# gau-nernst/llama-x

Hardware: AMD Instinct MI355X
Metric: train tokens/sec Llama-3.1-8B seq4096 at 1/2/4/8 MI355X; p50 step ms (higher is better)
Workload: dtype bf16; 1 GPU; Llama-3.1-8B text-only LoRA r=16 bf16, seq=4096, 1 sequence per GPU, causal mask, base+LM head frozen (BASELINE.json configs[1]); random-init weights at 8B dimensions; seq_len=4096, parallelism=dp1, launch=hipGraph replay (fwd+bwd+AdamW), lm_head_rows=labelled only

## Files before the change

llama-x_amd/csrc/attn.h:

```cpp
#pragma once
#include "common.h"
#include <type_traits>

#define BQ 128
#define BKV 64
#define TILE_BYTES (64 * HD * 2)

typedef __attribute__((address_space(3))) void lds_void;
typedef const __attribute__((address_space(1))) void gbl_void;
typedef __attribute__((address_space(3))) s16x4_t lds_s16x4;

static inline int attn_check_shape(const char* fn, int64_t B, int64_t S, int64_t H, int64_t KVH, int64_t head_dim) {
  LLX_REQUIRE(head_dim == HD, "%s: head_dim=%lld unsupported (only 128)", fn, (long long)head_dim);
  LLX_REQUIRE(B > 0 && S > 0 && H > 0 && KVH > 0 && H % KVH == 0, "%s: bad B/S/H/KVH", fn);
  return LLX_OK;
}
int attn_dropout_check(const char* fn, int64_t threshold, const void* rng, int64_t stream_id, int64_t B, int64_t H);
template <typename... K>
static inline hipError_t attn_lds_limit(int bytes, K... kernels) {
  hipError_t e = hipSuccess;
  for (const void* f : {(const void*)kernels...}) if (e == hipSuccess) e = hipFuncSetAttribute(f, hipFuncAttributeMaxDynamicSharedMemorySize, bytes);
  return e;
}
```

llama-x_amd/csrc/attn_bwd.hip:

```cpp
#include "attn.h"
#include "attn_dropout.h"

typedef __attribute__((ext_vector_type(8))) short s16x8_t;

__device__ __forceinline__ int dual_swz(int row) { return ((row & 3) << 2) | ((row >> 2) & 3); }
__device__ __forceinline__ uint32_t dual_swz(uint32_t row) { return ((row & 3) << 2) | ((row >> 2) & 3); }

__device__ __forceinline__ bf16x8_t tr_frag(const char* img, int row0, int db, int lane) {
  const int hh = lane >> 5, tq = (lane & 15) >> 2, tp = lane & 3, tsub = (lane >> 4) & 1;
  const int chunk = 4 * db + 2 * tsub + (tp >> 1);
  const int rlo = row0 + 4 * hh + tq, rhi = rlo + 8;
  s16x4_t lo = __builtin_amdgcn_ds_read_tr16_b64_v4i16((lds_s16x4*)(img + rlo * 256 + ((chunk ^ dual_swz(rlo)) << 4) + ((tp & 1) << 3)));
  s16x4_t hi = __builtin_amdgcn_ds_read_tr16_b64_v4i16((lds_s16x4*)(img + rhi * 256 + ((chunk ^ dual_swz(rhi)) << 4) + ((tp & 1) << 3)));
  s16x8_t v = {lo[0], lo[1], lo[2], lo[3], hi[0], hi[1], hi[2], hi[3]};
  return __builtin_bit_cast(bf16x8_t, v);
}

__device__ __forceinline__ bf16x8_t row_frag(const char* img, int row, int ks, int hh) {
  return *reinterpret_cast<const bf16x8_t*>(img + row * 256 + (((2 * ks + hh) ^ dual_swz(row)) << 4));
}

template <int N>
__device__ __forceinline__ void lds_tr_wait(s16x4_t& a, s16x4_t& b, s16x4_t (&c)[4], s16x4_t (&d)[4]) {
  asm volatile("s_waitcnt lgkmcnt(%10)"
               : "+v"(a), "+v"(b), "+v"(c[0]), "+v"(c[1]), "+v"(c[2]), "+v"(c[3]), "+v"(d[0]), "+v"(d[1]), "+v"(d[2]), "+v"(d[3])
               : "n"(N));
  __builtin_amdgcn_sched_barrier(0);
}
__device__ __forceinline__ uint32_t xor_imm(uint32_t a, int c) {
  if (c == 0) return a;
  uint32_t r;
  asm volatile("v_xor_b32 %0, %1, %2" : "=v"(r) : "n"(c), "v"(a));
  return r;
}

struct AttnBwdArgs {
  const bf16_t* q; const bf16_t* k; const bf16_t* v; const bf16_t* o; const bf16_t* d_o;
  const float* lse; float* delta; float* nlse;
  const float* rope;
  unsigned long long* stamps;
  bf16_t* dq; bf16_t* dk; bf16_t* dv;
  bf16_t* ds; int Sp;
  int64_t q_sb, q_ss, k_sb, k_ss, v_sb, v_ss, o_sb, o_ss, do_sb, do_ss;
  int64_t dq_sb, dq_ss, dk_sb, dk_ss, dv_sb, dv_ss;
  const int* doc_ids; const int* prefix_len; const uint8_t* flags;
  int B, S, H, KVH;
  float scale, scale_log2;
  const uint8_t* mask; int64_t m_sb, m_sq;
  const int64_t* rng; uint32_t drop_thr; float drop_c; int stream_id;
};

enum { BWD_CAUSAL = 0, BWD_RULE = 1, BWD_MASK = 2 };

__device__ __forceinline__ uint32_t mask_nibble(uint32_t w) {
  const uint32_t nz = (((w & 0x7f7f7f7fu) + 0x7f7f7f7fu) | w) & 0x80808080u;
  return ((nz >> 7) * 0x01020408u) >> 24;
}

#define DQ_STAGE_BYTES (2 * TILE_BYTES)
#define DQ_LDS_BYTES (2 * DQ_STAGE_BYTES)

template <int MODE, bool DROPOUT = false>
__global__ __launch_bounds__(256, 2) void attn_bwd_dq_kernel(const AttnBwdArgs a) {
  static_assert(!(DROPOUT && MODE == BWD_MASK), "dropout exists in the causal and the rule mode");
  constexpr bool GENERAL = MODE == BWD_RULE;
  constexpr bool FLAGS = MODE != BWD_CAUSAL;
  constexpr bool MASK = MODE == BWD_MASK;
  extern __shared__ __attribute__((aligned(256))) char smem[];
  const int tid = threadIdx.x, lane = tid & 63;
  const int wave = __builtin_amdgcn_readfirstlane(tid >> 6);
  const int nqb = (a.S + BQ - 1) / BQ, nkt = (a.S + BKV - 1) / BKV;
  const int qb = nqb - 1 - blockIdx.y;
  const int h = blockIdx.x, b = blockIdx.z;
  const int kvh = h / (a.H / a.KVH);
  const int r = lane & 31, hh = lane >> 5;
  const int qi = qb * BQ + wave * 32 + r;
  const int qrow = min(qi, a.S - 1);

  const uint8_t* fl = FLAGS ? a.flags + ((int64_t)b * nqb + qb) * nkt : nullptr;
  const int kt_end = FLAGS ? nkt : min(nkt, (qb * BQ + BQ + BKV - 1) / BKV);
  uint32_t fpack = 0;
  int fchunk = -1;
  auto tile_class = [&](int t) -> int {
    if constexpr (FLAGS) {
      if ((t >> 6) != fchunk) {
        fchunk = t >> 6;
        fpack = fl[min(fchunk * 64 + lane, nkt - 1)];
      }
      return __builtin_amdgcn_readlane((int)fpack, t & 63);
    } else {
      return (t * BKV + BKV - 1 <= qb * BQ) ? 2 : 1;
    }
  };
  auto next_tile = [&](int t) {
    while (t < kt_end && tile_class(t) == 0) ++t;
    return t;
  };

  const int srow_in = lane >> 4, sslot = lane & 15;
  const bf16_t* kbase = a.k + (int64_t)b * a.k_sb + kvh * HD;
  const bf16_t* vbase = a.v + (int64_t)b * a.v_sb + kvh * HD;
  uint32_t koff[4], voff[4];
#pragma unroll
  for (int i = 0; i < 4; ++i) {
    const int row = i * 16 + wave * 4 + srow_in;
    koff[i] = (uint32_t)(((int64_t)row * a.k_ss + (sslot ^ dual_swz(row)) * 8) * 2);
    voff[i] = (uint32_t)(((int64_t)row * a.v_ss + (sslot ^ (row & 15)) * 8) * 2);
  }
  auto stage = [&](int buf, int t) {
    char* sK = smem + buf * DQ_STAGE_BYTES;
    char* sV = sK + TILE_BYTES;
    if (t * BKV + BKV <= a.S) {
      const char* kt = (const char*)(kbase + (int64_t)t * BKV * a.k_ss);
      const char* vt = (const char*)(vbase + (int64_t)t * BKV * a.v_ss);
      if constexpr (DROPOUT) {
        uint32_t l0;
        asm volatile("v_mbcnt_lo_u32_b32 %0, -1, 0\n\tv_mbcnt_hi_u32_b32 %0, -1, %0" : "=v"(l0));
        const int slot = (int)(l0 & 15);
#pragma unroll
        for (int i = 0; i < 4; ++i) {
          const int row = i * 16 + wave * 4 + (int)(l0 >> 4);
          const uint32_t ko = (uint32_t)(((int64_t)row * a.k_ss + (slot ^ dual_swz(row)) * 8) * 2);
          const uint32_t vo = (uint32_t)(((int64_t)row * a.v_ss + (slot ^ (row & 15)) * 8) * 2);
          __builtin_amdgcn_global_load_lds((gbl_void*)(kt + ko), (lds_void*)(sK + (i * 16 + wave * 4) * 256), 16, 0, 0);
          __builtin_amdgcn_global_load_lds((gbl_void*)(vt + vo), (lds_void*)(sV + (i * 16 + wave * 4) * 256), 16, 0, 0);
        }
      } else {
#pragma unroll
      for (int i = 0; i < 4; ++i) {
        __builtin_amdgcn_global_load_lds((gbl_void*)(kt + koff[i]), (lds_void*)(sK + (i * 16 + wave * 4) * 256), 16, 0, 0);
        __builtin_amdgcn_global_load_lds((gbl_void*)(vt + voff[i]), (lds_void*)(sV + (i * 16 + wave * 4) * 256), 16, 0, 0);
      }
      }
    } else {
#pragma unroll
      for (int i = 0; i < 4; ++i) {
        const int row = i * 16 + wave * 4 + srow_in;
        const int key = min(t * BKV + row, a.S - 1);
        const int kc = sslot ^ dual_swz(row);
        const int vc = sslot ^ (row & 15);
        __builtin_amdgcn_global_load_lds((gbl_void*)(kbase + (int64_t)key * a.k_ss + kc * 8), (lds_void*)(sK + (i * 16 + wave * 4) * 256), 16, 0, 0);
        __builtin_amdgcn_global_load_lds((gbl_void*)(vbase + (int64_t)key * a.v_ss + vc * 8), (lds_void*)(sV + (i * 16 + wave * 4) * 256), 16, 0, 0);
      }
    }
  };

  const uint32_t sbase = (uint32_t)(uintptr_t)(__attribute__((address_space(3))) char*)smem;
  uint32_t aK0;
  {
    const int tq2 = (lane & 15) >> 2, tp = lane & 3, tsub = (lane >> 4) & 1;
    const int rlo = 4 * hh + tq2;
    aK0 = (uint32_t)(rlo * 256 + (((2 * tsub + (tp >> 1)) ^ dual_swz(rlo)) << 4) + ((tp & 1) << 3));
  }
  f32x16_t dq[4];
#pragma unroll
  for (int i = 0; i < 4; ++i)
#pragma unroll
    for (int e = 0; e < 16; ++e) dq[i][e] = 0.f;
  const int* docrow = (GENERAL && a.doc_ids) ? a.doc_ids + (int64_t)b * a.S : nullptr;
  const int my_doc = docrow ? docrow[qrow] : 0;
  const int my_prefix = (GENERAL && a.prefix_len) ? a.prefix_len[b] : 0;
  uint32_t mwn[MASK ? 8 : 1];
  auto mask_request = [&](int t_) {
    if constexpr (MASK) {
      uint32_t l0;
      asm volatile("v_mbcnt_lo_u32_b32 %0, -1, 0\n\tv_mbcnt_hi_u32_b32 %0, -1, %0" : "=v"(l0));
      const int hh = (int)(l0 >> 5);
      const uint8_t* mrow = a.mask + (int64_t)b * a.m_sb + (int64_t)min(qb * BQ + wave * 32 + (int)(l0 & 31), a.S - 1) * a.m_sq;
      if (t_ * BKV + BKV <= a.S) {
        const uint8_t* p = mrow + t_ * BKV + 4 * hh;
#pragma unroll
        for (int g = 0; g < 8; ++g) __builtin_memcpy(&mwn[g], p + (g >> 2) * 32 + 8 * (g & 3), 4);
      } else {
#pragma unroll
        for (int g = 0; g < 8; ++g) {
          const int g0 = t_ * BKV + (g >> 2) * 32 + 8 * (g & 3) + 4 * hh;
          __builtin_memcpy(&mwn[g], mrow + min(g0, a.S - 4), 4);
        }
      }
    }
  };
  auto mask_bits = [&](int t_) -> uint32_t {
    uint32_t bits = 0;
    if constexpr (MASK) {
      const bool ragged = t_ * BKV + BKV > a.S;
#pragma unroll
      for (int g = 0; g < 8; ++g) {
        uint32_t w = mwn[g];
        if (ragged) {
          const int g0 = t_ * BKV + (g >> 2) * 32 + 8 * (g & 3) + 4 * hh;
          const int sh = g0 - min(g0, a.S - 4);
          w = sh >= 4 ? 0u : w >> (8 * sh);
        }
        bits |= mask_nibble(w) << (4 * g);
      }
    }
    return bits;
  };

  int t = next_tile(0);
  if constexpr (MASK) {
#pragma unroll
    for (int g = 0; g < 8; ++g) mwn[g] = 0;
    if (t < kt_end && tile_class(t) == 1) mask_request(t);
  }
  if (t < kt_end) stage(0, t);
  bf16x8_t qf[8], dof[8], ovf[8];
  const float my_lse = a.lse[((int64_t)b * a.H + h) * a.S + qrow];
  {
    const bf16_t* qp = a.q + (int64_t)b * a.q_sb + (int64_t)qrow * a.q_ss + h * HD + 8 * hh;
    const bf16_t* dp = a.d_o + (int64_t)b * a.do_sb + (int64_t)qrow * a.do_ss + h * HD + 8 * hh;
    const bf16_t* op = a.o + (int64_t)b * a.o_sb + (int64_t)qrow * a.o_ss + h * HD + 8 * hh;
#pragma unroll
    for (int ks = 0; ks < 8; ++ks) {
      ovf[ks] = *reinterpret_cast<const bf16x8_t*>(op + 16 * ks);
      dof[ks] = *reinterpret_cast<const bf16x8_t*>(dp + 16 * ks);
      qf[ks] = *reinterpret_cast<const bf16x8_t*>(qp + 16 * ks);
    }
    __builtin_amdgcn_sched_barrier(0);
  }
  const float lse_safe = (my_lse == -INFINITY) ? 0.f : my_lse;
// ... 752 lines not shown
  return (2 * B * H * S + (H / KVH) * 2 * B * S * KVH * HD) * 4;
}

extern "C" int64_t llx_attn_bwd_ds_bytes(int64_t B, int64_t S, int64_t H) {
  const int64_t Sp = cdiv64(S, 256) * 256;
  return B * H * Sp * Sp * 2;
}

static int attn_bwd_set_attrs() {
  static const hipError_t e0 = attn_lds_limit(DQ_LDS_BYTES, attn_bwd_dq_kernel<BWD_CAUSAL>, attn_bwd_dq_kernel<BWD_RULE>, attn_bwd_dq_kernel<BWD_MASK>,
                                              attn_bwd_dq_kernel<BWD_CAUSAL, true>, attn_bwd_dq_kernel<BWD_RULE, true>);
  static const hipError_t e1 = attn_lds_limit(DQ2_LDS_BYTES, attn_bwd_dq2_kernel<false>, attn_bwd_dq2_kernel<true>);
  static const hipError_t e2 = attn_lds_limit(DKV3_LDS_BYTES, attn_bwd_dkv3_kernel<BWD_CAUSAL, false, false>, attn_bwd_dkv3_kernel<BWD_RULE, false, false>,
                                              attn_bwd_dkv3_kernel<BWD_MASK, false, false>, attn_bwd_dkv3_kernel<BWD_CAUSAL, true, false>,
                                              attn_bwd_dkv3_kernel<BWD_CAUSAL, false, true>, attn_bwd_dkv3_kernel<BWD_RULE, false, true>,
                                              attn_bwd_dkv3_kernel<BWD_CAUSAL, false, false, true>, attn_bwd_dkv3_kernel<BWD_RULE, false, false, true>);
  return e0 == hipSuccess && e1 == hipSuccess && e2 == hipSuccess ? LLX_OK : LLX_ERR_LAUNCH;
}

static int attn_bwd_args(const char* fn, AttnBwdArgs& a, const void* q, int64_t q_sb, int64_t q_ss, const void* k, int64_t k_sb, int64_t k_ss,
                         const void* v, int64_t v_sb, int64_t v_ss, const void* o, int64_t o_sb, int64_t o_ss, const void* d_o, int64_t do_sb,
                         int64_t do_ss, const float* lse, float* delta, void* dq, int64_t dq_sb, int64_t dq_ss, void* dk, int64_t dk_sb,
                         int64_t dk_ss, void* dv, int64_t dv_sb, int64_t dv_ss, const float* rope, int64_t B, int64_t S, int64_t H, int64_t KVH,
                         int64_t head_dim, float scale) {
  LLX_REQUIRE(q && k && v && o && d_o && lse && delta && dq && dk && dv, "%s: null pointer", fn);
  if (int rc = attn_check_shape(fn, B, S, H, KVH, head_dim)) return rc;
  LLX_REQUIRE(((q_ss | k_ss | v_ss | o_ss | do_ss | q_sb | k_sb | v_sb | o_sb | do_sb) % 8) == 0, "%s: input strides must keep 16-byte alignment", fn);
  LLX_REQUIRE(((dq_ss | dk_ss | dv_ss | dq_sb | dk_sb | dv_sb) % 4) == 0, "%s: output strides must keep 8-byte alignment", fn);
  LLX_REQUIRE(((uintptr_t)q | (uintptr_t)k | (uintptr_t)v | (uintptr_t)o | (uintptr_t)d_o) % 16 == 0, "%s: unaligned input", fn);
  LLX_REQUIRE(((uintptr_t)dq) % 8 == 0 && ((uintptr_t)dk | (uintptr_t)dv) % 16 == 0 && ((dk_ss | dv_ss | dk_sb | dv_sb) % 8) == 0,
              "%s: unaligned output", fn);
  LLX_REQUIRE(!rope || (uintptr_t)rope % 16 == 0, "%s: unaligned rope table", fn);
  LLX_REQUIRE(S < (1 << 24) && B * H < (1 << 16), "%s: S or B*H too large", fn);
  a = {};
  a.q = (const bf16_t*)q; a.k = (const bf16_t*)k; a.v = (const bf16_t*)v; a.o = (const bf16_t*)o; a.d_o = (const bf16_t*)d_o;
  a.lse = lse; a.delta = delta; a.nlse = delta + B * H * S; a.rope = rope; a.dq = (bf16_t*)dq; a.dk = (bf16_t*)dk; a.dv = (bf16_t*)dv;
  a.q_sb = q_sb; a.q_ss = q_ss; a.k_sb = k_sb; a.k_ss = k_ss; a.v_sb = v_sb; a.v_ss = v_ss; a.o_sb = o_sb; a.o_ss = o_ss;
  a.do_sb = do_sb; a.do_ss = do_ss; a.dq_sb = dq_sb; a.dq_ss = dq_ss; a.dk_sb = dk_sb; a.dk_ss = dk_ss; a.dv_sb = dv_sb; a.dv_ss = dv_ss;
  a.B = (int)B; a.S = (int)S; a.H = (int)H; a.KVH = (int)KVH;
  a.scale = scale; a.scale_log2 = scale * 1.4426950408889634f;
  return LLX_OK;
}

static int attn_bwd_dkv(const char* fn, void (*kernel)(const AttnBwdArgs, float*), const AttnBwdArgs& a, hipStream_t stream) {
  const int64_t B = a.B, S = a.S, H = a.H;
  float* part = a.nlse + B * H * S;
  hipLaunchKernelGGL(kernel, dim3((unsigned)(cdiv64(S, DKV2_KEYS) * B * H)), dim3(256), DKV3_LDS_BYTES, stream, a, part);
  LLX_LAUNCH_CHECK(fn);
  hipLaunchKernelGGL(attn_dkv_reduce_kernel, dim3((unsigned)cdiv64(B * S * a.KVH * HD / 8, 256)), dim3(256), 0, stream, a, (const float*)part);
  LLX_LAUNCH_CHECK(fn);
  return LLX_OK;
}

static int attn_bwd_run(const char* fn, const AttnBwdArgs& a, int mode, hipStream_t stream) {
  void (*const dq[5])(const AttnBwdArgs) = {attn_bwd_dq_kernel<BWD_CAUSAL>, attn_bwd_dq_kernel<BWD_RULE>, attn_bwd_dq_kernel<BWD_MASK>,
                                            attn_bwd_dq_kernel<BWD_CAUSAL, true>, attn_bwd_dq_kernel<BWD_RULE, true>};
  void (*const dkv[5])(const AttnBwdArgs, float*) = {attn_bwd_dkv3_kernel<BWD_CAUSAL, false, false>, attn_bwd_dkv3_kernel<BWD_RULE, false, false>,
                                                     attn_bwd_dkv3_kernel<BWD_MASK, false, false>, attn_bwd_dkv3_kernel<BWD_CAUSAL, false, false, true>,
                                                     attn_bwd_dkv3_kernel<BWD_RULE, false, false, true>};
  if (a.rng) mode += 3;
  if (attn_bwd_set_attrs() != LLX_OK) { llx_set_error("%s: cannot raise LDS limit", fn); return LLX_ERR_LAUNCH; }
  hipLaunchKernelGGL(dq[mode], dim3((unsigned)a.H, (unsigned)cdiv64(a.S, BQ), (unsigned)a.B), dim3(256), DQ_LDS_BYTES, stream, a);
  LLX_LAUNCH_CHECK(fn);
  return attn_bwd_dkv(fn, a.stamps ? attn_bwd_dkv3_kernel<BWD_CAUSAL, true, false> : dkv[mode], a, stream);
}

extern "C" int llx_attn_bwd(const void* q, int64_t q_sb, int64_t q_ss, const void* k, int64_t k_sb, int64_t k_ss, const void* v,
                            int64_t v_sb, int64_t v_ss, const void* o, int64_t o_sb, int64_t o_ss, const void* d_o, int64_t do_sb,
                            int64_t do_ss, const float* lse, float* delta, void* dq, int64_t dq_sb, int64_t dq_ss, void* dk,
                            int64_t dk_sb, int64_t dk_ss, void* dv, int64_t dv_sb, int64_t dv_ss, const int* doc_ids,
                            const int* prefix_len, const void* flags, const float* rope, void* ds, int64_t B, int64_t S, int64_t H,
                            int64_t KVH, int64_t head_dim, float scale, hipStream_t stream) {
  AttnBwdArgs a;
  if (int rc = attn_bwd_args("llx_attn_bwd", a, q, q_sb, q_ss, k, k_sb, k_ss, v, v_sb, v_ss, o, o_sb, o_ss, d_o, do_sb, do_ss, lse, delta, dq, dq_sb, dq_ss, dk,
                             dk_sb, dk_ss, dv, dv_sb, dv_ss, rope, B, S, H, KVH, head_dim, scale)) return rc;
  LLX_REQUIRE(!(doc_ids || prefix_len) || flags, "llx_attn_bwd: tile flags required with doc_ids/prefix_len");
  LLX_REQUIRE(!ds || (uintptr_t)ds % 256 == 0, "llx_attn_bwd: the dS buffer must be 256-byte aligned");
  a.doc_ids = doc_ids; a.prefix_len = prefix_len; a.flags = (doc_ids || prefix_len) ? (const uint8_t*)flags : nullptr;
  if (!ds || g_bwd_stamps || (a.flags && cdiv64(S, BKV) > 128)) {
    if (!a.flags) a.stamps = g_bwd_stamps;
    return attn_bwd_run("llx_attn_bwd", a, a.flags ? BWD_RULE : BWD_CAUSAL, stream);
  }
  if (attn_bwd_set_attrs() != LLX_OK) { llx_set_error("llx_attn_bwd: cannot raise LDS limit"); return LLX_ERR_LAUNCH; }
  a.ds = (bf16_t*)ds; a.Sp = (int)(cdiv64(S, 256) * 256);
  hipLaunchKernelGGL(attn_bwd_delta_kernel, dim3((unsigned)cdiv64(B * S * H, 16)), dim3(256), 0, stream, a);
  LLX_LAUNCH_CHECK("llx_attn_bwd(delta)");
  if (int rc = attn_bwd_dkv("llx_attn_bwd", a.flags ? attn_bwd_dkv3_kernel<BWD_RULE, false, true> : attn_bwd_dkv3_kernel<BWD_CAUSAL, false, true>, a, stream)) return rc;
  hipLaunchKernelGGL(a.flags ? attn_bwd_dq2_kernel<true> : attn_bwd_dq2_kernel<false>, dim3((unsigned)H, (unsigned)cdiv64(S, DQ2_BQ), (unsigned)B), dim3(512),
                     DQ2_LDS_BYTES, stream, a);
  LLX_LAUNCH_CHECK("llx_attn_bwd(dq from dS)");
  return LLX_OK;
}

extern "C" int llx_attn_mask_bwd(const void* q, int64_t q_sb, int64_t q_ss, const void* k, int64_t k_sb, int64_t k_ss, const void* v,
                                 int64_t v_sb, int64_t v_ss, const void* o, int64_t o_sb, int64_t o_ss, const void* d_o, int64_t do_sb,
                                 int64_t do_ss, const float* lse, float* delta, void* dq, int64_t dq_sb, int64_t dq_ss, void* dk,
                                 int64_t dk_sb, int64_t dk_ss, void* dv, int64_t dv_sb, int64_t dv_ss, const void* mask, int64_t m_sb,
                                 int64_t m_sq, const void* flags, const float* rope, int64_t B, int64_t S, int64_t H, int64_t KVH,
                                 int64_t head_dim, float scale, hipStream_t stream) {
  AttnBwdArgs a;
  if (int rc = attn_bwd_args("llx_attn_mask_bwd", a, q, q_sb, q_ss, k, k_sb, k_ss, v, v_sb, v_ss, o, o_sb, o_ss, d_o, do_sb, do_ss, lse, delta, dq, dq_sb, dq_ss, dk,
                             dk_sb, dk_ss, dv, dv_sb, dv_ss, rope, B, S, H, KVH, head_dim, scale)) return rc;
  LLX_REQUIRE(S >= 4, "llx_attn_mask_bwd: S=%lld (>= 4: the mask is read 4 bytes at a time)", (long long)S);
  LLX_REQUIRE(mask && flags, "llx_attn_mask_bwd: null pointer");
  LLX_REQUIRE(m_sq >= S && m_sb >= 0, "llx_attn_mask_bwd: mask rows overlap");
  a.flags = (const uint8_t*)flags; a.mask = (const uint8_t*)mask; a.m_sb = m_sb; a.m_sq = m_sq;
  return attn_bwd_run("llx_attn_mask_bwd", a, BWD_MASK, stream);
}

extern "C" int llx_attn_bwd_dropout(const void* q, int64_t q_sb, int64_t q_ss, const void* k, int64_t k_sb, int64_t k_ss, const void* v,
                                    int64_t v_sb, int64_t v_ss, const void* o, int64_t o_sb, int64_t o_ss, const void* d_o, int64_t do_sb,
                                    int64_t do_ss, const float* lse, float* delta, void* dq, int64_t dq_sb, int64_t dq_ss, void* dk,
                                    int64_t dk_sb, int64_t dk_ss, void* dv, int64_t dv_sb, int64_t dv_ss, const int* doc_ids,
                                    const int* prefix_len, const void* flags, const float* rope, void* ds, int64_t B, int64_t S, int64_t H,
                                    int64_t KVH, int64_t head_dim, float scale, int64_t threshold, const void* rng, int64_t stream_id,
// ... 12 lines not shown
```

llama-x_amd/csrc/attn_fwd.hip:

```cpp
#include "attn.h"
#include "attn_dropout.h"

#define KV_TILE_BYTES TILE_BYTES
#define ATT_STAGE_BYTES (2 * KV_TILE_BYTES)
#define ATT_LDS_BYTES (2 * ATT_STAGE_BYTES)

struct AttnFwdArgs {
  const bf16_t* q; const bf16_t* k; const bf16_t* v; bf16_t* o; float* lse;
  int64_t q_sb, q_ss, k_sb, k_ss, v_sb, v_ss, o_sb, o_ss;
  const int* doc_ids;
  const int* prefix_len;
  const uint8_t* flags;
  int B, S, H, KVH;
  float scale_log2;
  unsigned long long* stamps;
  int Skv;
  int64_t k_sh, v_sh;
  const uint8_t* mask;
  int64_t m_sb, m_sq;
  const int64_t* rng;
  uint32_t drop_thr;
  float drop_c;
  int stream_id;
};

enum { ATT_CAUSAL = 0, ATT_GENERAL = 1, ATT_MASK = 2 };

template <bool GENERAL_, bool STAMP = false, int NW = 8>
__global__ __launch_bounds__(64 * NW, 2) void attn_fwd_kernel(const AttnFwdArgs a) {
  static_assert(NW == 8, "NW stays a parameter only because bench.py, tools/ and profiles/ key on the symbol attn_fwd_kernel<*, *, 8>");
  constexpr int MODE = GENERAL_ ? ATT_GENERAL : ATT_CAUSAL;
  constexpr bool DROPOUT = false;
#include "attn_fwd_body.h"
}

template <bool GENERAL_>
__global__ __launch_bounds__(512, 2) void attn_fwd_dropout_kernel(const AttnFwdArgs a) {
  constexpr int MODE = GENERAL_ ? ATT_GENERAL : ATT_CAUSAL, NW = 8;
  constexpr bool STAMP = false, DROPOUT = true;
#include "attn_fwd_body.h"
}

__global__ __launch_bounds__(512, 2) void attn_mask_fwd_kernel(const AttnFwdArgs a) {
  constexpr int MODE = ATT_MASK, NW = 8;
  constexpr bool STAMP = false, DROPOUT = false;
#include "attn_fwd_body.h"
}

__global__ void attn_tile_flags_kernel(const int* __restrict__ doc_ids, const int* __restrict__ prefix_len, uint8_t* flags, int S,
                                       int nqb, int nkt) {
  __shared__ int s_any, s_all;
  const int kt = blockIdx.x, qb = blockIdx.y, b = blockIdx.z;
  if (threadIdx.x == 0) { s_any = 0; s_all = 1; }
  __syncthreads();
  const int P = prefix_len ? prefix_len[b] : 0;
  int any = 0, all = 1;
  for (int idx = threadIdx.x; idx < BQ * BKV; idx += blockDim.x) {
    const int qi = qb * BQ + idx / BKV, kk = kt * BKV + idx % BKV;
    if (qi >= S) continue;
    bool ok = (kk < S) && (kk <= qi || kk < P);
    if (ok && doc_ids) ok = doc_ids[(int64_t)b * S + qi] == doc_ids[(int64_t)b * S + kk];
    any |= ok; all &= ok;
  }
  if (any) atomicOr(&s_any, 1);
  if (!all) atomicAnd(&s_all, 0);
  __syncthreads();
  if (threadIdx.x == 0) flags[((int64_t)b * nqb + qb) * nkt + kt] = s_any ? (s_all ? 2 : 1) : 0;
}

extern "C" int64_t llx_attn_flags_bytes(int64_t B, int64_t S) { return B * cdiv64(S, BQ) * cdiv64(S, BKV); }

extern "C" int llx_attn_tile_flags(const int* doc_ids, const int* prefix_len, void* flags, int64_t B, int64_t S, hipStream_t stream) {
  LLX_REQUIRE(flags && B > 0 && S > 0, "llx_attn_tile_flags: bad arguments");
  const int nqb = (int)cdiv64(S, BQ), nkt = (int)cdiv64(S, BKV);
  hipLaunchKernelGGL(attn_tile_flags_kernel, dim3(nkt, nqb, (unsigned)B), dim3(256), 0, stream, doc_ids, prefix_len, (uint8_t*)flags,
                     (int)S, nqb, nkt);
  LLX_LAUNCH_CHECK("llx_attn_tile_flags");
  return LLX_OK;
}

static int attn_fwd_args(const char* fn, AttnFwdArgs& a, const void* q, int64_t q_sb, int64_t q_ss, const void* k, int64_t k_sb, int64_t k_ss,
                         const void* v, int64_t v_sb, int64_t v_ss, void* o, int64_t o_sb, int64_t o_ss, float* lse, int64_t B, int64_t S,
                         int64_t H, int64_t KVH, int64_t head_dim, float scale) {
  LLX_REQUIRE(q && k && v && o, "%s: null pointer", fn);
  if (int rc = attn_check_shape(fn, B, S, H, KVH, head_dim)) return rc;
  LLX_REQUIRE((q_ss % 8 | k_ss % 8 | v_ss % 8 | o_ss % 4 | q_sb % 8 | k_sb % 8 | v_sb % 8 | o_sb % 4) == 0, "%s: strides must keep 16-byte alignment", fn);
  LLX_REQUIRE(((uintptr_t)q | (uintptr_t)k | (uintptr_t)v) % 16 == 0 && (uintptr_t)o % 8 == 0, "%s: unaligned pointer", fn);
  a = {};
  a.q = (const bf16_t*)q; a.k = (const bf16_t*)k; a.v = (const bf16_t*)v; a.o = (bf16_t*)o; a.lse = lse;
  a.q_sb = q_sb; a.q_ss = q_ss; a.k_sb = k_sb; a.k_ss = k_ss; a.v_sb = v_sb; a.v_ss = v_ss; a.o_sb = o_sb; a.o_ss = o_ss;
  a.B = (int)B; a.S = (int)S; a.H = (int)H; a.KVH = (int)KVH;
  a.scale_log2 = scale * 1.4426950408889634f;
  return LLX_OK;
}

static int attn_fwd_launch(const char* fn, void (*kernel)(const AttnFwdArgs), const AttnFwdArgs& a, hipStream_t stream) {
  static const hipError_t err = attn_lds_limit(ATT_LDS_BYTES, attn_fwd_kernel<false, false, 8>, attn_fwd_kernel<true, false, 8>,
                                               attn_fwd_kernel<false, true, 8>, attn_mask_fwd_kernel, attn_fwd_dropout_kernel<false>,
                                               attn_fwd_dropout_kernel<true>);
  if (err != hipSuccess) { llx_set_error("%s: %s", fn, hipGetErrorString(err)); return LLX_ERR_LAUNCH; }
  hipLaunchKernelGGL(kernel, dim3((unsigned)a.H, (unsigned)cdiv64(a.S, 256), (unsigned)a.B), dim3(512), ATT_LDS_BYTES, stream, a);
  LLX_LAUNCH_CHECK(fn);
  return LLX_OK;
}

extern "C" int llx_attn_fwd(const void* q, int64_t q_sb, int64_t q_ss, const void* k, int64_t k_sb, int64_t k_ss, const void* v,
                            int64_t v_sb, int64_t v_ss, void* o, int64_t o_sb, int64_t o_ss, float* lse, const int* doc_ids,
                            const int* prefix_len, const void* flags, int64_t B, int64_t S, int64_t H, int64_t KVH, int64_t head_dim,
                            float scale, hipStream_t stream) {
  AttnFwdArgs a;
  if (int rc = attn_fwd_args("llx_attn_fwd", a, q, q_sb, q_ss, k, k_sb, k_ss, v, v_sb, v_ss, o, o_sb, o_ss, lse, B, S, H, KVH, head_dim, scale)) return rc;
  LLX_REQUIRE(!(doc_ids || prefix_len) || flags, "llx_attn_fwd: tile flags required with doc_ids/prefix_len");
  a.doc_ids = doc_ids; a.prefix_len = prefix_len; a.flags = (doc_ids || prefix_len) ? (const uint8_t*)flags : nullptr;
  LLX_REQUIRE(S < (1 << 24), "llx_attn_fwd: S too large");
  return attn_fwd_launch("llx_attn_fwd", a.flags ? attn_fwd_kernel<true, false, 8> : attn_fwd_kernel<false, false, 8>, a, stream);
}

int attn_dropout_check(const char* fn, int64_t threshold, const void* rng, int64_t stream_id, int64_t B, int64_t H) {
  LLX_REQUIRE(rng && (uintptr_t)rng % 8 == 0, "%s: rng must be a device pointer to two int64 (seed, counter)", fn);
  LLX_REQUIRE(threshold > 0 && threshold < 65536, "%s: threshold=%lld out of range (0 < round(p * 65536) < 65536)", fn, (long long)threshold);
  LLX_REQUIRE(stream_id >= 0 && stream_id < (1ll << 31), "%s: stream_id=%lld out of range", fn, (long long)stream_id);
  LLX_REQUIRE(B < 65536 && H < 65536, "%s: B and H must stay below 65536 (the mask key takes 16 bits of each)", fn);
  return LLX_OK;
}

extern "C" int llx_attn_fwd_dropout(const void* q, int64_t q_sb, int64_t q_ss, const void* k, int64_t k_sb, int64_t k_ss, const void* v,
                                    int64_t v_sb, int64_t v_ss, void* o, int64_t o_sb, int64_t o_ss, float* lse, const int* doc_ids,
                                    const int* prefix_len, const void* flags, int64_t B, int64_t S, int64_t H, int64_t KVH, int64_t head_dim,
                                    float scale, int64_t threshold, const void* rng, int64_t stream_id, hipStream_t stream) {
  AttnFwdArgs a;
  if (int rc = attn_fwd_args("llx_attn_fwd_dropout", a, q, q_sb, q_ss, k, k_sb, k_ss, v, v_sb, v_ss, o, o_sb, o_ss, lse, B, S, H, KVH, head_dim, scale)) return rc;
  if (int rc = attn_dropout_check("llx_attn_fwd_dropout", threshold, rng, stream_id, B, H)) return rc;
  LLX_REQUIRE(!(doc_ids || prefix_len) || flags, "llx_attn_fwd_dropout: tile flags required with doc_ids/prefix_len");
  LLX_REQUIRE(S < (1 << 24), "llx_attn_fwd_dropout: S too large");
  a.doc_ids = doc_ids; a.prefix_len = prefix_len; a.flags = (doc_ids || prefix_len) ? (const uint8_t*)flags : nullptr;
  a.rng = (const int64_t*)rng; a.drop_thr = (uint32_t)threshold << 16; a.drop_c = 65536.f / (float)(65536 - threshold); a.stream_id = (int)stream_id;
  return attn_fwd_launch("llx_attn_fwd_dropout", a.flags ? attn_fwd_dropout_kernel<true> : attn_fwd_dropout_kernel<false>, a, stream);
}

__global__ __launch_bounds__(256) void attn_dropout_keep_kernel(uint8_t* __restrict__ keep, const int64_t* __restrict__ rng, int stream_id,
                                                               uint32_t thr16, int H, int Sq, int Skv, int64_t total) {
  const int64_t idx = (int64_t)blockIdx.x * 256 + threadIdx.x;
  if (idx >= total) return;
  const int k = (int)(idx % Skv);
  int64_t r = idx / Skv;
  const int q = (int)(r % Sq);
  r /= Sq;
  keep[idx] = attn_dropout_keep(rng[0], rng[1], stream_id, (int)(r / H), (int)(r % H), q, k, thr16) ? 1 : 0;
}

extern "C" int llx_attn_dropout_keep(void* keep, int64_t B, int64_t H, int64_t Sq, int64_t Skv, int64_t threshold, const void* rng,
                                     int64_t stream_id, hipStream_t stream) {
  LLX_REQUIRE(keep && B > 0 && H > 0 && Sq > 0 && Skv > 0, "llx_attn_dropout_keep: bad arguments");
  if (int rc = attn_dropout_check("llx_attn_dropout_keep", threshold, rng, stream_id, B, H)) return rc;
  LLX_REQUIRE(Sq < (1 << 24) && Skv < (1 << 24), "llx_attn_dropout_keep: Sq or Skv too large");
  const int64_t total = B * H * Sq * Skv;
  LLX_REQUIRE(cdiv64(total, 256) < (1ll << 31), "llx_attn_dropout_keep: too many elements");
  hipLaunchKernelGGL(attn_dropout_keep_kernel, dim3((unsigned)cdiv64(total, 256)), dim3(256), 0, stream, (uint8_t*)keep, (const int64_t*)rng,
                     (int)stream_id, (uint32_t)threshold << 16, (int)H, (int)Sq, (int)Skv, total);
  LLX_LAUNCH_CHECK("llx_attn_dropout_keep");
  return LLX_OK;
}

__global__ __launch_bounds__(256) void attn_mask_tile_flags_kernel(const uint8_t* __restrict__ mask, int64_t m_sb, int64_t m_sq,
                                                                  uint8_t* __restrict__ flags, int Sq, int Skv, int nqb, int nkt) {
  __shared__ int s_any, s_all;
  const int kt = blockIdx.x, qb = blockIdx.y, b = blockIdx.z;
  if (threadIdx.x == 0) { s_any = 0; s_all = 1; }
  __syncthreads();
  const uint8_t* mb = mask + (int64_t)b * m_sb;
  const int n_in = min(BKV, Skv - kt * BKV);
  int any = 0, all = (n_in == BKV);
  for (int idx = threadIdx.x; idx < BQ * (BKV / 4); idx += blockDim.x) {
    const int qi = qb * BQ + idx / (BKV / 4), g0 = kt * BKV + 4 * (idx % (BKV / 4));
    if (qi >= Sq || g0 >= Skv) continue;
    const int off = min(g0, Skv - 4), n = min(4, Skv - g0);
    uint32_t w;
    __builtin_memcpy(&w, mb + (int64_t)qi * m_sq + off, 4);
    w >>= 8 * (g0 - off);
    int cnt = 0;
#pragma unroll
    for (int i = 0; i < 4; ++i) cnt += (i < n && ((w >> (8 * i)) & 0xffu) != 0) ? 1 : 0;
    any |= cnt > 0; all &= cnt == n;
  }
  if (any) atomicOr(&s_any, 1);
  if (!all) atomicAnd(&s_all, 0);
  __syncthreads();
  if (threadIdx.x == 0) flags[((int64_t)b * nqb + qb) * nkt + kt] = s_any ? (s_all ? 2 : 1) : 0;
}

extern "C" int64_t llx_attn_mask_flags_bytes(int64_t B, int64_t Sq, int64_t Skv) { return B * cdiv64(Sq, BQ) * cdiv64(Skv, BKV); }

extern "C" int llx_attn_mask_tile_flags(const void* mask, int64_t m_sb, int64_t m_sq, void* flags, int64_t B, int64_t Sq, int64_t Skv,
                                        hipStream_t stream) {
  LLX_REQUIRE(mask && flags && B > 0 && Sq > 0, "llx_attn_mask_tile_flags: bad arguments");
  LLX_REQUIRE(Skv >= 4 && Skv < (1 << 24) && Sq < (1 << 24) && B < 65536, "llx_attn_mask_tile_flags: Skv=%lld (>= 4) / Sq=%lld / B=%lld out of range",
              (long long)Skv, (long long)Sq, (long long)B);
  LLX_REQUIRE(m_sq >= Skv && m_sb >= 0, "llx_attn_mask_tile_flags: mask rows overlap");
  const int nqb = (int)cdiv64(Sq, BQ), nkt = (int)cdiv64(Skv, BKV);
  hipLaunchKernelGGL(attn_mask_tile_flags_kernel, dim3(nkt, nqb, (unsigned)B), dim3(256), 0, stream, (const uint8_t*)mask, m_sb, m_sq,
                     (uint8_t*)flags, (int)Sq, (int)Skv, nqb, nkt);
  LLX_LAUNCH_CHECK("llx_attn_mask_tile_flags");
  return LLX_OK;
}

extern "C" int llx_attn_mask_fwd(const void* q, int64_t q_sb, int64_t q_ss, const void* k, int64_t k_sb, int64_t k_sh, int64_t k_ss,
                                 const void* v, int64_t v_sb, int64_t v_sh, int64_t v_ss, void* o, int64_t o_sb, int64_t o_ss, float* lse,
                                 const void* mask, int64_t m_sb, int64_t m_sq, const void* flags, int64_t B, int64_t Sq, int64_t Skv,
                                 int64_t H, int64_t KVH, int64_t head_dim, float scale, hipStream_t stream) {
  AttnFwdArgs a;
  if (int rc = attn_fwd_args("llx_attn_mask_fwd", a, q, q_sb, q_ss, k, k_sb, k_ss, v, v_sb, v_ss, o, o_sb, o_ss, lse, B, Sq, H, KVH, head_dim, scale)) return rc;
  LLX_REQUIRE(B < 65536, "llx_attn_mask_fwd: bad B/Sq/H/KVH");
  LLX_REQUIRE(Skv >= 4 && Skv < (1 << 24) && Sq < (1 << 24), "llx_attn_mask_fwd: Skv=%lld (>= 4) / Sq=%lld out of range", (long long)Skv, (long long)Sq);
  LLX_REQUIRE((k_sh % 8 | v_sh % 8) == 0, "llx_attn_mask_fwd: strides must keep 16-byte alignment");
  LLX_REQUIRE(k_ss >= 0 && v_ss >= 0 && k_ss < (1 << 24) && v_ss < (1 << 24), "llx_attn_mask_fwd: K/V position stride out of range");
  LLX_REQUIRE(mask && flags, "llx_attn_mask_fwd: null pointer");
  LLX_REQUIRE(m_sq >= Skv && m_sb >= 0, "llx_attn_mask_fwd: mask rows overlap");
  a.flags = (const uint8_t*)flags; a.Skv = (int)Skv; a.k_sh = k_sh; a.v_sh = v_sh; a.mask = (const uint8_t*)mask; a.m_sb = m_sb; a.m_sq = m_sq;
  return attn_fwd_launch("llx_attn_mask_fwd", attn_mask_fwd_kernel, a, stream);
}

extern "C" int llx_debug_attn_fwd_occupancy(void) {
  int n = -1;
  hipFuncSetAttribute((const void*)attn_fwd_kernel<false, false, 8>, hipFuncAttributeMaxDynamicSharedMemorySize, ATT_LDS_BYTES);
  hipError_t e = hipOccupancyMaxActiveBlocksPerMultiprocessor(&n, (const void*)attn_fwd_kernel<false, false, 8>, 512, ATT_LDS_BYTES);
  if (e != hipSuccess) { llx_set_error("occupancy query: %s", hipGetErrorString(e)); return -1; }
  return n;
}

extern "C" int llx_debug_attn_fwd_stamps(const void* q, const void* k, const void* v, void* o, int64_t S, int64_t H, int64_t KVH,
                                         unsigned long long* stamps, hipStream_t stream) {
  AttnFwdArgs a;
  if (int rc = attn_fwd_args("llx_debug_attn_fwd_stamps", a, q, S * H * HD, H * HD, k, S * KVH * HD, KVH * HD, v, S * KVH * HD, KVH * HD, o,
                             S * H * HD, H * HD, nullptr, 1, S, H, KVH, HD, 0.08838834764f)) return rc;
  a.stamps = stamps;
  return attn_fwd_launch("llx_debug_attn_fwd_stamps", attn_fwd_kernel<false, true, 8>, a, stream);
}
```

llama-x_amd/csrc/attn_fwd_body.h:

```cpp
  constexpr bool GENERAL = MODE != ATT_CAUSAL;
  constexpr bool DOCS = MODE == ATT_GENERAL;
  constexpr bool MASK = MODE == ATT_MASK;
  constexpr int WQ = 32 * NW;
  constexpr int NP = 16 / NW;
  extern __shared__ __attribute__((aligned(16))) char smem[];
  const int tid = threadIdx.x, lane = tid & 63;
  const int wave = __builtin_amdgcn_readfirstlane(tid >> 6);
  int SK = a.S;
  if constexpr (MASK) SK = a.Skv;
  const int nqb = (a.S + BQ - 1) / BQ, nkt = (SK + BKV - 1) / BKV;
  const int nwb = (a.S + WQ - 1) / WQ;
  const int qb = nwb - 1 - blockIdx.y;
  const int h = blockIdx.x, b = blockIdx.z;
  const int kvh = h / (a.H / a.KVH);
  const int r = lane & 31, hh = lane >> 5;
  const int qi = qb * WQ + wave * 32 + r;
  const int q_lo = qb * WQ + wave * 32;
  const int qrow = min(qi, a.S - 1);

  bf16x8_t qf[8];
  {
    const bf16_t* qp = a.q + (int64_t)b * a.q_sb + (int64_t)qrow * a.q_ss + h * HD + 8 * hh;
#pragma unroll
    for (int ks = 0; ks < 8; ++ks) qf[ks] = *reinterpret_cast<const bf16x8_t*>(qp + 16 * ks);
  }

  const int my_qb = min((qb * WQ + wave * 32) / BQ, nqb - 1);
  const uint8_t* fl = GENERAL ? a.flags + ((int64_t)b * nqb + my_qb) * nkt : nullptr;
  const uint8_t* fl0 = GENERAL ? a.flags + ((int64_t)b * nqb + min(qb * WQ / BQ, nqb - 1)) * nkt : nullptr;
  const uint8_t* fl1 = GENERAL ? a.flags + ((int64_t)b * nqb + min(qb * WQ / BQ + 1, nqb - 1)) * nkt : nullptr;
  const int kt_end = GENERAL ? nkt : min(nkt, (qb * WQ + WQ + BKV - 1) / BKV);
  uint32_t fpack = 0;
  int fchunk = -1;
  auto flags_of = [&](int t) -> uint32_t {
    if ((t >> 6) != fchunk) {
      fchunk = t >> 6;
      const int idx = min(fchunk * 64 + lane, nkt - 1);
      fpack = (uint32_t)fl[idx] | ((uint32_t)fl0[idx] << 8) | ((uint32_t)fl1[idx] << 16);
    }
    return (uint32_t)__builtin_amdgcn_readlane((int)fpack, t & 63);
  };
  auto tile_class = [&](int t) -> int {
    if constexpr (GENERAL) return (int)(flags_of(t) & 0xff);
    else return (t * BKV > q_lo + 31) ? 0 : ((t * BKV + BKV - 1 <= q_lo) ? 2 : 1);
  };
  auto next_tile = [&](int t) {
    if constexpr (GENERAL) while (t < kt_end && (flags_of(t) >> 8) == 0) ++t;
    return t;
  };

  const int srow_in = lane >> 4, sslot = lane & 15;
  const bf16_t* kbase = a.k + (int64_t)b * a.k_sb + kvh * HD;
  const bf16_t* vbase = a.v + (int64_t)b * a.v_sb + kvh * HD;
  if constexpr (MASK) {
    kbase = a.k + (int64_t)b * a.k_sb + (int64_t)kvh * a.k_sh;
    vbase = a.v + (int64_t)b * a.v_sb + (int64_t)kvh * a.v_sh;
  }
  uint32_t koff[NP], voff[NP];
#pragma unroll
  for (int i = 0; i < NP; ++i) {
    const int row = (i * NW + wave) * 4 + srow_in;
    koff[i] = (uint32_t)(((int64_t)row * a.k_ss + (sslot ^ (row & 15)) * 8) * 2);
    voff[i] = (uint32_t)(((int64_t)row * a.v_ss + (sslot ^ ((row & 3) << 2)) * 8) * 2);
  }
  auto stage = [&](int buf, int t) {
    char* sK = smem + buf * ATT_STAGE_BYTES;
    char* sV = sK + KV_TILE_BYTES;
    if (t * BKV + BKV <= SK) {
      const char* kt = (const char*)(kbase + (int64_t)t * BKV * a.k_ss);
      const char* vt = (const char*)(vbase + (int64_t)t * BKV * a.v_ss);
#pragma unroll
      for (int i = 0; i < NP; ++i) {
        __builtin_amdgcn_global_load_lds((gbl_void*)(kt + koff[i]), (lds_void*)(sK + (i * NW + wave) * 1024), 16, 0, 0);
        __builtin_amdgcn_global_load_lds((gbl_void*)(vt + voff[i]), (lds_void*)(sV + (i * NW + wave) * 1024), 16, 0, 0);
      }
    } else {
#pragma unroll
      for (int i = 0; i < NP; ++i) {
        const int row = (i * NW + wave) * 4 + srow_in;
        const int key = min(t * BKV + row, SK - 1);
        const int kc = sslot ^ (row & 15);
        const int vc = sslot ^ ((row & 3) << 2);
        __builtin_amdgcn_global_load_lds((gbl_void*)(kbase + (int64_t)key * a.k_ss + kc * 8), (lds_void*)(sK + (i * NW + wave) * 1024), 16, 0, 0);
// ... 244 lines not shown
```

Baseline: 32070 tokens/s.

## Pack GQA query heads per workgroup in attention dq backward and general forward

```diff
diff --git a/llama-x_amd/csrc/attn.h b/llama-x_amd/csrc/attn.h
--- a/llama-x_amd/csrc/attn.h
+++ b/llama-x_amd/csrc/attn.h
@@ -15,6 +15,7 @@
   LLX_REQUIRE(B > 0 && S > 0 && H > 0 && KVH > 0 && H % KVH == 0, "%s: bad B/S/H/KVH", fn);
   return LLX_OK;
 }
+static inline int attn_gqa_pack_log2(int G) { return G == 2 ? 1 : G == 4 ? 2 : G == 8 ? 3 : 0; }
 int attn_dropout_check(const char* fn, int64_t threshold, const void* rng, int64_t stream_id, int64_t B, int64_t H);
 template <typename... K>
 static inline hipError_t attn_lds_limit(int bytes, K... kernels) {
diff --git a/llama-x_amd/csrc/attn_bwd.hip b/llama-x_amd/csrc/attn_bwd.hip
--- a/llama-x_amd/csrc/attn_bwd.hip
+++ b/llama-x_amd/csrc/attn_bwd.hip
@@ -48,6 +48,7 @@
   float scale, scale_log2;
   const uint8_t* mask; int64_t m_sb, m_sq;
   const int64_t* rng; uint32_t drop_thr; float drop_c; int stream_id;
+  int gps;
 };
 
 enum { BWD_CAUSAL = 0, BWD_RULE = 1, BWD_MASK = 2 };
@@ -59,9 +60,10 @@
 
 #define DQ_STAGE_BYTES (2 * TILE_BYTES)
 #define DQ_LDS_BYTES (2 * DQ_STAGE_BYTES)
+#define DQ_PIECE(i) (8 * ((i) & 1) + 4 * ((i) >> 1))
 
 template <int MODE, bool DROPOUT = false>
-__global__ __launch_bounds__(256, 2) void attn_bwd_dq_kernel(const AttnBwdArgs a) {
+__global__ __launch_bounds__(512, 2) void attn_bwd_dq_kernel(const AttnBwdArgs a) {
   static_assert(!(DROPOUT && MODE == BWD_MASK), "dropout exists in the causal and the rule mode");
   constexpr bool GENERAL = MODE == BWD_RULE;
   constexpr bool FLAGS = MODE != BWD_CAUSAL;
@@ -70,15 +72,19 @@
   const int tid = threadIdx.x, lane = tid & 63;
   const int wave = __builtin_amdgcn_readfirstlane(tid >> 6);
   const int nqb = (a.S + BQ - 1) / BQ, nkt = (a.S + BKV - 1) / BKV;
-  const int qb = nqb - 1 - blockIdx.y;
-  const int h = blockIdx.x, b = blockIdx.z;
+  const int gps = MODE == BWD_CAUSAL ? a.gps : 0;
+  const int WQ = 256 >> (gps ? gps : 1);
+  const int qb = (a.S + WQ - 1) / WQ - 1 - blockIdx.y;
+  const int wh = gps ? wave >> (3 - gps) : 0, wr = gps ? wave & ((8 >> gps) - 1) : wave;
+  const int h = (blockIdx.x << gps) + wh, b = blockIdx.z;
   const int kvh = h / (a.H / a.KVH);
   const int r = lane & 31, hh = lane >> 5;
-  const int qi = qb * BQ + wave * 32 + r;
+  const int q_lo = qb * WQ + wr * 32;
+  const int qi = q_lo + r;
   const int qrow = min(qi, a.S - 1);
 
-  const uint8_t* fl = FLAGS ? a.flags + ((int64_t)b * nqb + qb) * nkt : nullptr;
-  const int kt_end = FLAGS ? nkt : min(nkt, (qb * BQ + BQ + BKV - 1) / BKV);
+  const uint8_t* fl = FLAGS ? a.flags + ((int64_t)b * nqb + qb * WQ / BQ) * nkt : nullptr;
+  const int kt_end = FLAGS ? nkt : min(nkt, (qb * WQ + WQ + BKV - 1) / BKV);
   uint32_t fpack = 0;
   int fchunk = -1;
   auto tile_class = [&](int t) -> int {
@@ -89,7 +95,7 @@
       }
       return __builtin_amdgcn_readlane((int)fpack, t & 63);
     } else {
-      return (t * BKV + BKV - 1 <= qb * BQ) ? 2 : 1;
+      return (t * BKV + BKV - 1 <= qb * WQ) ? 2 : 1;
     }
   };
   auto next_tile = [&](int t) {
@@ -100,12 +106,12 @@
   const int srow_in = lane >> 4, sslot = lane & 15;
   const bf16_t* kbase = a.k + (int64_t)b * a.k_sb + kvh * HD;
   const bf16_t* vbase = a.v + (int64_t)b * a.v_sb + kvh * HD;
-  uint32_t koff[4], voff[4];
-#pragma unroll
-  for (int i = 0; i < 4; ++i) {
-    const int row = i * 16 + wave * 4 + srow_in;
-    koff[i] = (uint32_t)(((int64_t)row * a.k_ss + (sslot ^ dual_swz(row)) * 8) * 2);
-    voff[i] = (uint32_t)(((int64_t)row * a.v_ss + (sslot ^ (row & 15)) * 8) * 2);
+  const bool np4 = gps == 0;
+  uint32_t koff, voff;
+  {
+    const int row = wave * 4 + srow_in;
+    koff = (uint32_t)(((int64_t)row * a.k_ss + (sslot ^ dual_swz(row)) * 8) * 2);
+    voff = (uint32_t)(((int64_t)row * a.v_ss + (sslot ^ (row & 15)) * 8) * 2);
   }
   auto stage = [&](int buf, int t) {
     char* sK = smem + buf * DQ_STAGE_BYTES;
@@ -114,33 +120,45 @@
       const char* kt = (const char*)(kbase + (int64_t)t * BKV * a.k_ss);
       const char* vt = (const char*)(vbase + (int64_t)t * BKV * a.v_ss);
       if constexpr (DROPOUT) {
-        uint32_t l0;
-        asm volatile("v_mbcnt_lo_u32_b32 %0, -1, 0\n\tv_mbcnt_hi_u32_b32 %0, -1, %0" : "=v"(l0));
-        const int slot = (int)(l0 & 15);
+        auto pair = [&](auto i0_tag) {
+          constexpr int i0 = decltype(i0_tag)::value;
+          uint32_t l0;
+          asm volatile("v_mbcnt_lo_u32_b32 %0, -1, 0\n\tv_mbcnt_hi_u32_b32 %0, -1, %0" : "=v"(l0));
+          const int slot = (int)(l0 & 15);
+#pragma unroll
+          for (int i = i0; i < i0 + 2; ++i) {
+            const int row = (DQ_PIECE(i) + wave) * 4 + (int)(l0 >> 4);
+            const uint32_t ko = (uint32_t)(((int64_t)row * a.k_ss + (slot ^ dual_swz(row)) * 8) * 2);
+            const uint32_t vo = (uint32_t)(((int64_t)row * a.v_ss + (slot ^ (row & 15)) * 8) * 2);
+            __builtin_amdgcn_global_load_lds((gbl_void*)(kt + ko), (lds_void*)(sK + (DQ_PIECE(i) + wave) * 1024), 16, 0, 0);
+            __builtin_amdgcn_global_load_lds((gbl_void*)(vt + vo), (lds_void*)(sV + (DQ_PIECE(i) + wave) * 1024), 16, 0, 0);
+          }
+        };
+        pair(std::integral_constant<int, 0>{});
+        if (np4) pair(std::integral_constant<int, 2>{});
+      } else {
 #pragma unroll
         for (int i = 0; i < 4; ++i) {
-          const int row = i * 16 + wave * 4 + (int)(l0 >> 4);
-          const uint32_t ko = (uint32_t)(((int64_t)row * a.k_ss + (slot ^ dual_swz(row)) * 8) * 2);
-          const uint32_t vo = (uint32_t)(((int64_t)row * a.v_ss + (slot ^ (row & 15)) * 8) * 2);
-          __builtin_amdgcn_global_load_lds((gbl_void*)(kt + ko), (lds_void*)(sK + (i * 16 + wave * 4) * 256), 16, 0, 0);
-          __builtin_amdgcn_global_load_lds((gbl_void*)(vt + vo), (lds_void*)(sV + (i * 16 + wave * 4) * 256), 16, 0, 0);
-        }
-      } else {
+          if (i == 2 && !np4) break;
+          const char* kp = kt + (int64_t)(8 * DQ_PIECE(i)) * a.k_ss;
+          const char* vp = vt + (int64_t)(8 * DQ_PIECE(i)) * a.v_ss;
+          __builtin_amdgcn_global_load_lds((gbl_void*)(kp + koff), (lds_void*)(sK + (DQ_PIECE(i) + wave) * 1024), 16, 0, 0);
+          __builtin_amdgcn_global_load_lds((gbl_void*)(vp + voff), (lds_void*)(sV + (DQ_PIECE(i) + wave) * 1024), 16, 0, 0);
+        }
+      }
+    } else {
+      uint32_t l0;
+      asm volatile("v_mbcnt_lo_u32_b32 %0, -1, 0\n\tv_mbcnt_hi_u32_b32 %0, -1, %0" : "=v"(l0));
+      const int slot = (int)(l0 & 15);
 #pragma unroll
       for (int i = 0; i < 4; ++i) {
-        __builtin_amdgcn_global_load_lds((gbl_void*)(kt + koff[i]), (lds_void*)(sK + (i * 16 + wave * 4) * 256), 16, 0, 0);
-        __builtin_amdgcn_global_load_lds((gbl_void*)(vt + voff[i]), (lds_void*)(sV + (i * 16 + wave * 4) * 256), 16, 0, 0);
-      }
-      }
-    } else {
-#pragma unroll
-      for (int i = 0; i < 4; ++i) {
-        const int row = i * 16 + wave * 4 + srow_in;
+        if (i == 2 && !np4) break;
+        const int row = (DQ_PIECE(i) + wave) * 4 + (int)(l0 >> 4);
         const int key = min(t * BKV + row, a.S - 1);
-        const int kc = sslot ^ dual_swz(row);
-        const int vc = sslot ^ (row & 15);
-        __builtin_amdgcn_global_load_lds((gbl_void*)(kbase + (int64_t)key * a.k_ss + kc * 8), (lds_void*)(sK + (i * 16 + wave * 4) * 256), 16, 0, 0);
-        __builtin_amdgcn_global_load_lds((gbl_void*)(vbase + (int64_t)key * a.v_ss + vc * 8), (lds_void*)(sV + (i * 16 + wave * 4) * 256), 16, 0, 0);
+        const int kc = slot ^ dual_swz(row);
+        const int vc = slot ^ (row & 15);
+        __builtin_amdgcn_global_load_lds((gbl_void*)(kbase + (int64_t)key * a.k_ss + kc * 8), (lds_void*)(sK + (DQ_PIECE(i) + wave) * 1024), 16, 0, 0);
+        __builtin_amdgcn_global_load_lds((gbl_void*)(vbase + (int64_t)key * a.v_ss + vc * 8), (lds_void*)(sV + (DQ_PIECE(i) + wave) * 1024), 16, 0, 0);
       }
     }
   };
@@ -166,7 +184,7 @@
       uint32_t l0;
       asm volatile("v_mbcnt_lo_u32_b32 %0, -1, 0\n\tv_mbcnt_hi_u32_b32 %0, -1, %0" : "=v"(l0));
       const int hh = (int)(l0 >> 5);
-      const uint8_t* mrow = a.mask + (int64_t)b * a.m_sb + (int64_t)min(qb * BQ + wave * 32 + (int)(l0 & 31), a.S - 1) * a.m_sq;
+      const uint8_t* mrow = a.mask + (int64_t)b * a.m_sb + (int64_t)min(q_lo + (int)(l0 & 31), a.S - 1) * a.m_sq;
       if (t_ * BKV + BKV <= a.S) {
         const uint8_t* p = mrow + t_ * BKV + 4 * hh;
 #pragma unroll
@@ -1025,7 +1043,7 @@
   return LLX_OK;
 }
 
-static int attn_bwd_run(const char* fn, const AttnBwdArgs& a, int mode, hipStream_t stream) {
+static int attn_bwd_run(const char* fn, AttnBwdArgs a, int mode, hipStream_t stream) {
   void (*const dq[5])(const AttnBwdArgs) = {attn_bwd_dq_kernel<BWD_CAUSAL>, attn_bwd_dq_kernel<BWD_RULE>, attn_bwd_dq_kernel<BWD_MASK>,
                                             attn_bwd_dq_kernel<BWD_CAUSAL, true>, attn_bwd_dq_kernel<BWD_RULE, true>};
   void (*const dkv[5])(const AttnBwdArgs, float*) = {attn_bwd_dkv3_kernel<BWD_CAUSAL, false, false>, attn_bwd_dkv3_kernel<BWD_RULE, false, false>,
@@ -1033,7 +1051,10 @@
                                                      attn_bwd_dkv3_kernel<BWD_RULE, false, false, true>};
   if (a.rng) mode += 3;
   if (attn_bwd_set_attrs() != LLX_OK) { llx_set_error("%s: cannot raise LDS limit", fn); return LLX_ERR_LAUNCH; }
-  hipLaunchKernelGGL(dq[mode], dim3((unsigned)a.H, (unsigned)cdiv64(a.S, BQ), (unsigned)a.B), dim3(256), DQ_LDS_BYTES, stream, a);
+  a.gps = a.flags ? 0 : attn_gqa_pack_log2(a.H / a.KVH);
+  const int dq_rows = a.gps ? 256 >> a.gps : BQ;
+  hipLaunchKernelGGL(dq[mode], dim3((unsigned)(a.H >> a.gps), (unsigned)cdiv64(a.S, dq_rows), (unsigned)a.B), dim3(a.gps ? 512 : 256), DQ_LDS_BYTES,
+                     stream, a);
   LLX_LAUNCH_CHECK(fn);
   return attn_bwd_dkv(fn, a.stamps ? attn_bwd_dkv3_kernel<BWD_CAUSAL, true, false> : dkv[mode], a, stream);
 }
diff --git a/llama-x_amd/csrc/attn_fwd.hip b/llama-x_amd/csrc/attn_fwd.hip
--- a/llama-x_amd/csrc/attn_fwd.hip
+++ b/llama-x_amd/csrc/attn_fwd.hip
@@ -22,6 +22,7 @@
   uint32_t drop_thr;
   float drop_c;
   int stream_id;
+  int gps;
 };
 
 enum { ATT_CAUSAL = 0, ATT_GENERAL = 1, ATT_MASK = 2 };
@@ -31,6 +32,7 @@
   static_assert(NW == 8, "NW stays a parameter only because bench.py, tools/ and profiles/ key on the symbol attn_fwd_kernel<*, *, 8>");
   constexpr int MODE = GENERAL_ ? ATT_GENERAL : ATT_CAUSAL;
   constexpr bool DROPOUT = false;
+  const int GPS = GENERAL_ ? a.gps : 0;
 #include "attn_fwd_body.h"
 }
 
@@ -38,11 +40,12 @@
 __global__ __launch_bounds__(512, 2) void attn_fwd_dropout_kernel(const AttnFwdArgs a) {
   constexpr int MODE = GENERAL_ ? ATT_GENERAL : ATT_CAUSAL, NW = 8;
   constexpr bool STAMP = false, DROPOUT = true;
+  const int GPS = GENERAL_ ? a.gps : 0;
 #include "attn_fwd_body.h"
 }
 
 __global__ __launch_bounds__(512, 2) void attn_mask_fwd_kernel(const AttnFwdArgs a) {
-  constexpr int MODE = ATT_MASK, NW = 8;
+  constexpr int MODE = ATT_MASK, NW = 8, GPS = 0;
   constexpr bool STAMP = false, DROPOUT = false;
 #include "attn_fwd_body.h"
 }
@@ -94,12 +97,13 @@
   return LLX_OK;
 }
 
-static int attn_fwd_launch(const char* fn, void (*kernel)(const AttnFwdArgs), const AttnFwdArgs& a, hipStream_t stream) {
+static int attn_fwd_launch(const char* fn, void (*kernel)(const AttnFwdArgs), AttnFwdArgs a, bool pack, hipStream_t stream) {
   static const hipError_t err = attn_lds_limit(ATT_LDS_BYTES, attn_fwd_kernel<false, false, 8>, attn_fwd_kernel<true, false, 8>,
                                                attn_fwd_kernel<false, true, 8>, attn_mask_fwd_kernel, attn_fwd_dropout_kernel<false>,
                                                attn_fwd_dropout_kernel<true>);
   if (err != hipSuccess) { llx_set_error("%s: %s", fn, hipGetErrorString(err)); return LLX_ERR_LAUNCH; }
-  hipLaunchKernelGGL(kernel, dim3((unsigned)a.H, (unsigned)cdiv64(a.S, 256), (unsigned)a.B), dim3(512), ATT_LDS_BYTES, stream, a);
+  a.gps = pack ? attn_gqa_pack_log2(a.H / a.KVH) : 0;
+  hipLaunchKernelGGL(kernel, dim3((unsigned)(a.H >> a.gps), (unsigned)cdiv64(a.S, 256 >> a.gps), (unsigned)a.B), dim3(512), ATT_LDS_BYTES, stream, a);
   LLX_LAUNCH_CHECK(fn);
   return LLX_OK;
 }
@@ -113,7 +117,7 @@
   LLX_REQUIRE(!(doc_ids || prefix_len) || flags, "llx_attn_fwd: tile flags required with doc_ids/prefix_len");
   a.doc_ids = doc_ids; a.prefix_len = prefix_len; a.flags = (doc_ids || prefix_len) ? (const uint8_t*)flags : nullptr;
   LLX_REQUIRE(S < (1 << 24), "llx_attn_fwd: S too large");
-  return attn_fwd_launch("llx_attn_fwd", a.flags ? attn_fwd_kernel<true, false, 8> : attn_fwd_kernel<false, false, 8>, a, stream);
+  return attn_fwd_launch("llx_attn_fwd", a.flags ? attn_fwd_kernel<true, false, 8> : attn_fwd_kernel<false, false, 8>, a, a.flags != nullptr, stream);
 }
 
 int attn_dropout_check(const char* fn, int64_t threshold, const void* rng, int64_t stream_id, int64_t B, int64_t H) {
@@ -135,7 +139,7 @@
   LLX_REQUIRE(S < (1 << 24), "llx_attn_fwd_dropout: S too large");
   a.doc_ids = doc_ids; a.prefix_len = prefix_len; a.flags = (doc_ids || prefix_len) ? (const uint8_t*)flags : nullptr;
   a.rng = (const int64_t*)rng; a.drop_thr = (uint32_t)threshold << 16; a.drop_c = 65536.f / (float)(65536 - threshold); a.stream_id = (int)stream_id;
-  return attn_fwd_launch("llx_attn_fwd_dropout", a.flags ? attn_fwd_dropout_kernel<true> : attn_fwd_dropout_kernel<false>, a, stream);
+  return attn_fwd_launch("llx_attn_fwd_dropout", a.flags ? attn_fwd_dropout_kernel<true> : attn_fwd_dropout_kernel<false>, a, a.flags != nullptr, stream);
 }
 
 __global__ __launch_bounds__(256) void attn_dropout_keep_kernel(uint8_t* __restrict__ keep, const int64_t* __restrict__ rng, int stream_id,
@@ -217,7 +221,7 @@
   LLX_REQUIRE(mask && flags, "llx_attn_mask_fwd: null pointer");
   LLX_REQUIRE(m_sq >= Skv && m_sb >= 0, "llx_attn_mask_fwd: mask rows overlap");
   a.flags = (const uint8_t*)flags; a.Skv = (int)Skv; a.k_sh = k_sh; a.v_sh = v_sh; a.mask = (const uint8_t*)mask; a.m_sb = m_sb; a.m_sq = m_sq;
-  return attn_fwd_launch("llx_attn_mask_fwd", attn_mask_fwd_kernel, a, stream);
+  return attn_fwd_launch("llx_attn_mask_fwd", attn_mask_fwd_kernel, a, false, stream);
 }
 
 extern "C" int llx_debug_attn_fwd_occupancy(void) {
@@ -234,5 +238,5 @@
   if (int rc = attn_fwd_args("llx_debug_attn_fwd_stamps", a, q, S * H * HD, H * HD, k, S * KVH * HD, KVH * HD, v, S * KVH * HD, KVH * HD, o,
                              S * H * HD, H * HD, nullptr, 1, S, H, KVH, HD, 0.08838834764f)) return rc;
   a.stamps = stamps;
-  return attn_fwd_launch("llx_debug_attn_fwd_stamps", attn_fwd_kernel<false, true, 8>, a, stream);
-}
+  return attn_fwd_launch("llx_debug_attn_fwd_stamps", attn_fwd_kernel<false, true, 8>, a, false, stream);
+}
diff --git a/llama-x_amd/csrc/attn_fwd_body.h b/llama-x_amd/csrc/attn_fwd_body.h
--- a/llama-x_amd/csrc/attn_fwd_body.h
+++ b/llama-x_amd/csrc/attn_fwd_body.h
@@ -1,7 +1,7 @@
   constexpr bool GENERAL = MODE != ATT_CAUSAL;
   constexpr bool DOCS = MODE == ATT_GENERAL;
   constexpr bool MASK = MODE == ATT_MASK;
-  constexpr int WQ = 32 * NW;
+  const int WQ = (32 * NW) >> GPS;
   constexpr int NP = 16 / NW;
   extern __shared__ __attribute__((aligned(16))) char smem[];
   const int tid = threadIdx.x, lane = tid & 63;
@@ -11,11 +11,13 @@
   const int nqb = (a.S + BQ - 1) / BQ, nkt = (SK + BKV - 1) / BKV;
   const int nwb = (a.S + WQ - 1) / WQ;
   const int qb = nwb - 1 - blockIdx.y;
-  const int h = blockIdx.x, b = blockIdx.z;
+  const int wh = GPS ? wave >> (__builtin_ctz(NW) - GPS) : 0;
+  const int wr = GPS ? wave & ((NW >> GPS) - 1) : wave;
+  const int h = (blockIdx.x << GPS) + wh, b = blockIdx.z;
   const int kvh = h / (a.H / a.KVH);
   const int r = lane & 31, hh = lane >> 5;
-  const int qi = qb * WQ + wave * 32 + r;
-  const int q_lo = qb * WQ + wave * 32;
+  const int qi = qb * WQ + wr * 32 + r;
+  const int q_lo = qb * WQ + wr * 32;
   const int qrow = min(qi, a.S - 1);
 
   bf16x8_t qf[8];
@@ -25,10 +27,10 @@
     for (int ks = 0; ks < 8; ++ks) qf[ks] = *reinterpret_cast<const bf16x8_t*>(qp + 16 * ks);
   }
 
-  const int my_qb = min((qb * WQ + wave * 32) / BQ, nqb - 1);
+  const int my_qb = min(q_lo / BQ, nqb - 1);
   const uint8_t* fl = GENERAL ? a.flags + ((int64_t)b * nqb + my_qb) * nkt : nullptr;
   const uint8_t* fl0 = GENERAL ? a.flags + ((int64_t)b * nqb + min(qb * WQ / BQ, nqb - 1)) * nkt : nullptr;
-  const uint8_t* fl1 = GENERAL ? a.flags + ((int64_t)b * nqb + min(qb * WQ / BQ + 1, nqb - 1)) * nkt : nullptr;
+  const uint8_t* fl1 = GENERAL ? a.flags + ((int64_t)b * nqb + min(qb * WQ / BQ + (GPS ? 0 : 1), nqb - 1)) * nkt : nullptr;
   const int kt_end = GENERAL ? nkt : min(nkt, (qb * WQ + WQ + BKV - 1) / BKV);
   uint32_t fpack = 0;
   int fchunk = -1;
```

New measurement: 32020 tokens/s (median of 2 runs). About the same (-0.1%).
